# puzzlepaint/surfelmeshing

Measured on AMD Instinct MI355X. Metric: RGB-D frames/s integrated @640x480, 5M live surfels; achieved HBM GB/s, higher is better.
Workload: dtype f32; 1 GPU; C2: synthetic room stream 640x480, raw depth + colour frames resident in HBM, full preprocessing + Integrate per frame, 4912850 live surfels (6250000 slots), steady-state re-traversal; max_surfel_count=6250000, streams=1, parallelism=1 independent stream per GPU

## Files before the change

### surfelmeshing_amd/csrc/smx_recon.hip

```cpp
#include <math.h>
#include <cmath>
#include <stdlib.h>
#include <string.h>

#include <algorithm>
#include <atomic>
#include <vector>

#include "smx_recon_state.hpp"
#include "smx_mesh.hpp"
#include <hip/hip_ext.h>

using namespace smx;

namespace {

struct FrameCtx {
  Mat34 L;
  Mat34 G;
  float fx, fy, cx, cy;
  Unproj up;
  float inv_depth_scaling;
  float sensor_noise_factor;
  float cos_normal_compat;
// ... 634 lines not shown
    have[q] = k < n_binned;
    pr[q] = tb.pairs[(size_t)tile * tb.cap + (have[q] ? k : 0u)];
  }
#pragma unroll
  for (int q = 0; q < kPairCache; ++q) { keep(pr[q].x); keep(pr[q].y); if (!have[q]) pr[q] = make_uint2(0u, 0u); }
  const uint16_t own_depth = in_image ? depth(y, x) : (uint16_t)0;
  const float2 own_normal = in_image ? normals(y, x) : make_float2(0.f, 0.f);
  PairRec rec[kPairCache];
#pragma unroll
  for (int q = 0; q < kPairCache; ++q) rec[q] = fetch_pair(S, c, pr[q].x, pr[q].y);
  t.zmin[lane] = 0x7F800000;
  t.sup[lane] = kInvalid; t.cnt[lane] = 0; t.confl[lane] = kInvalid; t.sum[lane] = 0;
  t.depth[lane] = own_depth; t.nrm[lane] = own_normal;
  __syncthreads();
  SMX_STAMP(stamps, 1);
  auto zmin_stage = [&](const PairRec& r) { if (r.code & kPairActive) atomicMin(&t.zmin[r.code & 255u], __float_as_int(r.l.z)); };
#pragma unroll
  for (int q = 0; q < kPairCache; ++q) if (have[q]) zmin_stage(rec[q]);
  for_uncached_pairs(S, c, tb, tile, n_binned, overflowed, n_ovf, zmin_stage);
  __syncthreads();
  SMX_STAMP(stamps, 2);
  if (lane == 0) {
    tb.count[tile * kCountStride] = 0;
    if (tile == 0) { *next_ovf_count = 0; seg_work_count[0] = 0; seg_work_count[1] = 0; }
    if (c.stats) {
      atomicAdd(&st->n_pairs, n_total);
      atomicMax(&st->max_tile_pairs, n_total);
      if (tile == 0) st->n_overflow_pairs = n_ovf;
    }
  }
#pragma unroll
  for (int q = 0; q < kPairCache; ++q) if (have[q]) assoc_stage(t, c, rec[q]);
  for_uncached_pairs(S, c, tb, tile, n_binned, overflowed, n_ovf, [&](const PairRec& r) { assoc_stage(t, c, r); });
  __syncthreads();
  SMX_STAMP(stamps, 3);
  uint32_t cand[kPairCache];
  float4 cp4[kPairCache], cn4[kPairCache];
#pragma unroll
  for (int q = 0; q < kPairCache; ++q) cand[q] = have[q] ? merge_candidate(t, c, rec[q]) : kInvalid;
#pragma unroll
  for (int q = 0; q < kPairCache; ++q) {
    const uint32_t g = cand[q] == kInvalid ? 0u : cand[q];
    cp4[q] = *S.group(kGroupP, g); cn4[q] = *S.group(kGroupN, g);
  }
#pragma unroll
  for (int q = 0; q < kPairCache; ++q) { keep(cp4[q]); keep(cn4[q]); }
#pragma unroll
  for (int q = 0; q < kPairCache; ++q) if (cand[q] != kInvalid) merge_decide(rec[q], cp4[q], cn4[q], merge_flag);
  for_uncached_pairs(S, c, tb, tile, n_binned, overflowed, n_ovf, [&](const PairRec& r) { merge_stage(t, S, c, r, merge_flag); });
  __syncthreads();
  SMX_STAMP(stamps, 4);
  if (in_image) {
    const size_t k = (size_t)y * c.W + x;
    sc.first_depth[k] = __int_as_float(t.zmin[lane]);
    sc.supporting[k] = t.sup[lane];
    sc.counts[k] = t.cnt[lane];
    sc.depth_sums[k] = (long long)t.sum[lane];
    sc.confl_key[k] = t.confl[lane];
  }
  SMX_STAMP(stamps, 5);
  ts_end(c.ts, kTsTilesEnd, blockIdx.x, gridDim.x);
}

__device__ __forceinline__ float depth_sum_avg(const Scratch& sc, size_t k) {
  return q_to_float(sc.depth_sums[k]) / (float)sc.counts[k];
}

__global__ void __launch_bounds__(kBlock)
k_blend_start(float ds, Img<uint16_t> depth, Scratch sc, BlendBufs b, int W, int H, unsigned long long* ts) {
  ts_end(ts, kTsBlendEnd, blockIdx.y * gridDim.x + blockIdx.x, gridDim.x * gridDim.y);
  const int x = blockIdx.x * 64 + (threadIdx.x & 63);
  const int y = blockIdx.y * 4 + (threadIdx.x >> 6);
  if (!(x >= 1 && y >= 1 && x < W - 1 && y < H - 1)) return;
  const size_t k = (size_t)y * W + x;
  const uint16_t own = depth(y, x);
  if (own == 0 || sc.supporting[k] == kInvalid) return;
  bool measurement_border = false, surfel_border = false;
  for (int wy = y - 1; wy <= y + 1; ++wy)
    for (int wx = x - 1; wx <= x + 1; ++wx) {
      if (depth(wy, wx) == 0) measurement_border = true;
      else if (sc.supporting[(size_t)wy * W + wx] == kInvalid) surfel_border = true;
    }
  if (surfel_border) {
    b.new_distance_map[k] = 1;
    const float avg = depth_sum_avg(sc, k);
    b.new_deltas[k] = avg - (float)own / ds;
  }
  if (measurement_border) {
    b.distance_map[k] = 1;
    const float avg = depth_sum_avg(sc, k);
    b.deltas[k] = avg - (float)own / ds;
    depth(y, x) = f2u16(ds * avg + 0.5f);
  } else {
    b.distance_map[k] = 255;
  }
}

__global__ void __launch_bounds__(kBlock)
k_blend_iter(int it, float term, float ds, Img<uint16_t> depth, Scratch sc, BlendBufs b, int W, int H, unsigned long long* ts) {
  ts_end(ts, kTsBlendEnd, blockIdx.y * gridDim.x + blockIdx.x, gridDim.x * gridDim.y);
  const int x = blockIdx.x * 64 + (threadIdx.x & 63);
  const int y = blockIdx.y * 4 + (threadIdx.x >> 6);
  if (!(x >= 1 && y >= 1 && x < W - 1 && y < H - 1)) return;
  const size_t k = (size_t)y * W + x;
  if (b.distance_map[k] == 255) {
    float delta_sum = 0; int count = 0;
    for (int wy = y - 1; wy <= y + 1; ++wy)
// ... 279 lines not shown
    const int k = min(k0 + j, P - 1);
    const int y = k / W, x = k - y * W;
    dv[j] = depth(y, x); sv[j] = sc.supporting[k]; cv[j] = sc.confl_key[k];
  }
#pragma unroll
  for (int j = 0; j < kScanPxPerThread; ++j) { keep(dv[j]); keep(sv[j]); keep(cv[j]); }
#pragma unroll
  for (int j = 0; j < kScanPxPerThread; ++j) {
    const int k = k0 + j;
    bool fl = false;
    if (k < P) {
      const int y = k / W, x = k - y * W;
      const uint16_t d = (uint16_t)dv[j];
      if (copy_back) depth_out(y, x) = d;
      fl = x >= 1 && y >= 1 && x < W - 1 && y < H - 1 && d > 0 && sv[j] == kInvalid && cv[j] == kInvalid;
      flags[k] = fl ? 1 : 0;
    }
    f[j] = fl ? 1u : 0u;
    mine += f[j];
  }
  const uint32_t lane = threadIdx.x & 63, wave = threadIdx.x >> 6;
  uint32_t incl = mine;
#pragma unroll
  for (int off = 1; off < 64; off <<= 1) {
    const uint32_t t = __shfl_up(incl, off);
    if (lane >= (uint32_t)off) incl += t;
  }
  if (lane == 63) wave_tot[wave] = incl;
  __syncthreads();
  uint32_t wave_off = 0, total = 0;
#pragma unroll
  for (int w = 0; w < kBlock / 64; ++w) {
    if ((uint32_t)w < wave) wave_off += wave_tot[w];
    total += wave_tot[w];
  }
  uint32_t run = wave_off + incl - mine;
#pragma unroll
  for (int j = 0; j < kScanPxPerThread; ++j) {
    const int k = k0 + j;
    if (k < P) local_rank[k] = run;
    run += f[j];
  }
  if (threadIdx.x == 0) {
    block_sums[block] = total;
    if (block == 0) st->create_base_next = st->surfel_count;
  }
}

struct FrameIn {
  Img<const uint16_t> depth; Img<const float2> normals; Img<const float> radius; Img<const uchar3> color;
};

struct PixelIn {
  uint16_t depth; float first; uint32_t key; uint32_t count; float2 nxy; uchar3 col; float radius;
};
__device__ __forceinline__ PixelIn load_pixel(const FrameCtx& c, const Scratch& sc, const FrameIn& in, int x, int y) {
  const size_t k = (size_t)y * c.W + x;
  PixelIn p;
  p.depth = in.depth(y, x); p.first = sc.first_depth[k]; p.key = sc.confl_key[k]; p.count = sc.counts[k];
  p.nxy = in.normals(y, x); p.col = in.color(y, x); p.radius = in.radius(y, x);
  return p;
}

__device__ __forceinline__ void keep(const PixelIn& p) {
  keep((uint32_t)p.depth); keep(p.first); keep(p.key); keep(p.count); keep(p.nxy); keep(p.radius);
  keep((uint32_t)p.col.x | ((uint32_t)p.col.y << 8) | ((uint32_t)p.col.z << 16));
}

struct SurfelRegs {
  float4 P;
  float4 N;
  float4 C;
  bool dirty;
  bool replaced;
  Vec3 new_smooth;
};

__device__ __forceinline__ void integrate_or_conflict(SurfelRegs& R, const FrameCtx& c, const PixelIn& px,
                                                      bool integrate, int x, int y,
                                                      const Vec3& cam, uint32_t i, DevState* st) {
  if (!integrate) return;
  const float measurement_depth = c.inv_depth_scaling * (float)px.depth;
  if (measurement_depth <= 0) return;
  bool conflicting = false;
  const float first = px.first;
  if (first < (1 - c.sensor_noise_factor) * measurement_depth) {
    if (first == cam.z) {
      const uint32_t key = px.key;
      if (key != kInvalid && (key & 0x7FFFFFFFu) == i) conflicting = true;
    }
    integrate = false;
  }
  if (!integrate && !conflicting) return;
  const float occlusion_depth = (1 + c.sensor_noise_factor) * measurement_depth;
  if (cam.z > occlusion_depth) integrate = false;
  if (!integrate && !conflicting) return;

  const float depth = measurement_depth;
  const Vec3 lp = {depth * (c.up.fx_inv * (float)x + c.up.cx_inv), depth * (c.up.fy_inv * (float)y + c.up.cy_inv), depth};
  const Vec3 gp = mul(c.G, lp);
  const float2 nxy = px.nxy;
  const Vec3 mn = {nxy.x, nxy.y, meas_normal_z(nxy.x, nxy.y)};
  const Vec3 gn = rotate(c.G, mn);
  const uchar3 col = px.col;

  if (conflicting) {
    if (c.stats) atomicAdd(&st->n_conflict_hits, 1u);
    float confidence = R.C.x;
    confidence -= 1;
    R.dirty = true;
    if (confidence <= 0) {
      if (c.stats) atomicAdd(&st->n_replaced, 1u);
      R.P = make_float4(gp.x, gp.y, gp.z, __uint_as_float(c.frame));
      R.new_smooth = gp;
      R.replaced = true;
      R.N = make_float4(gn.x, gn.y, gn.z, px.radius);
      R.C = make_float4(1.0f, __uint_as_float(c.frame),
                        __uint_as_float((uint32_t)col.x | ((uint32_t)col.y << 8) | ((uint32_t)col.z << 16) | (1u << 24)), R.C.w);
    } else {
      R.C.x = confidence;
    }
  }
  if (!integrate) return;

  const float surfel_distance = sqrtf(cam.x * cam.x + cam.y * cam.y + cam.z * cam.z);
  const Vec3 sn = {R.N.x, R.N.y, R.N.z};
  const Vec3 ln = rotate(c.L, sn);
  const float dot_angle = (1.0f / surfel_distance) * (cam.x * ln.x + cam.y * ln.y + cam.z * ln.z);
  if (dot_angle > 0) return;
  if (measurement_depth < cam.z) {
    const float d = sn.x * gn.x + sn.y * gn.y + sn.z * gn.z;
    if (d < c.cos_normal_compat) integrate = false;
  }
  const float old_r2 = R.N.w;
  if (old_r2 < 0) integrate = false;
  if (!integrate) return;

  uint32_t cnt = px.count;
  if (cnt < 1) cnt = 1;
  const float weight = 1.0f / (float)cnt;
  if (__float_as_uint(R.C.y) < c.frame) {
    if (c.stats) atomicAdd(&st->n_integrated, 1u);
    const float confidence = R.C.x;
    R.C.x = (confidence + weight < c.max_conf) ? (confidence + weight) : c.max_conf;
    const float nf = 1.0f / (confidence + weight);
    R.P.x = (confidence * R.P.x + weight * gp.x) * nf;
    R.P.y = (confidence * R.P.y + weight * gp.y) * nf;
    R.P.z = (confidence * R.P.z + weight * gp.z) * nf;
    const Vec3 nn = {confidence * sn.x + weight * gn.x, confidence * sn.y + weight * gn.y, confidence * sn.z + weight * gn.z};
    const float inv = 1.0f / sqrtf(nn.x * nn.x + nn.y * nn.y + nn.z * nn.z);
    R.N = make_float4(inv * nn.x, inv * nn.y, inv * nn.z, fminf(old_r2, px.radius));
    const uint32_t oc = __float_as_uint(R.C.z);
    const uint32_t c0 = (uint32_t)(uint8_t)(int)((confidence * (float)(oc & 255u) + weight * (float)col.x) * nf + 0.5f);
    const uint32_t c1 = (uint32_t)(uint8_t)(int)((confidence * (float)((oc >> 8) & 255u) + weight * (float)col.y) * nf + 0.5f);
    const uint32_t c2 = (uint32_t)(uint8_t)(int)((confidence * (float)((oc >> 16) & 255u) + weight * (float)col.z) * nf + 0.5f);
    R.C.z = __uint_as_float(c0 | (c1 << 8) | (c2 << 16));
    R.P.w = __uint_as_float(c.frame);
    R.dirty = true;
  }
}

template <bool kUseList>
__global__ void __launch_bounds__(kBlock)
k_integrate(Surfels S, FrameCtx c, Scratch sc, FrameIn in, Lists L,
            uint8_t* __restrict__ merge_flag, DevState* st, NewFlagsArgs nf, uint32_t n_flag_blocks) {
  SMX_SET_WAVE_PRIO();
#ifdef SMX_STAMPS
  if (nf.dbg && blockIdx.x == 0 && threadIdx.x == 0) nf.dbg[0] = wall_clock64();
#endif
  if (blockIdx.x < n_flag_blocks) { ts_begin(c.ts, kTsIntBegin); new_flags_scan_body(nf, sc, c.W, c.H, st, blockIdx.x); return; }
  const uint32_t block = blockIdx.x - n_flag_blocks, n_blocks = gridDim.x - n_flag_blocks;
  const uint32_t n_scan = kUseList ? 0u : st->surfel_count;
  uint32_t merged_here = 0;
  uint32_t ent, cntv;
  const uint32_t n_steps = vis_begin<kUseList>(L, n_scan, block, ent, cntv);
  for (uint32_t w = block; w < n_steps; w += n_blocks) {
    const uint32_t cur = ent;
    ent = (w + n_blocks < n_steps) ? vis_load<kUseList>(L, w + n_blocks) : 0u;
    uint32_t i;
    if (!vis_entry<kUseList>(cur, w, cntv, n_scan, threadIdx.x, i)) continue;
    const uint32_t merge_mark = merge_flag[i];
    SurfelRegs R;
    R.P = *S.group(kGroupP, i); R.N = *S.group(kGroupN, i); R.C = *S.group(kGroupC, i);
    if (merge_mark) {
      merge_flag[i] = 0;
      S.u(kLastUpdateStamp, i) = 0;
      S.f(kRadiusSq, i) = -1;
      const uint32_t col = (__float_as_uint(R.C.z) & 0x00FFFFFFu) | 0x01000000u;
      S.u(kColor, i) = col;
      L.flags8[i] = make_flags(0u, col, c.frame, c.reg_window);
      L.hot_epoch[i >> L.hot_shift] = (uint8_t)L.epoch;
      if (L.dirty8) L.dirty8[i] = 1;
      ++merged_here;
      continue;
    }
    R.dirty = false; R.replaced = false;
    const float4 p4 = R.P, n4 = R.N;
    if (!is_active(__float_as_uint(p4.w), c.frame, c.window)) continue;
    Proj p;
    const Vec3 g = {p4.x, p4.y, p4.z};
    if (!project_pos(g, c, p)) continue;
    if (n4.w < 0) continue;
    int ox = p.px, oy = p.py;
    const bool second = quadrant(p, c, ox, oy);
    const PixelIn px0 = load_pixel(c, sc, in, p.px, p.py);
    const PixelIn px1 = load_pixel(c, sc, in, ox, oy);
    integrate_or_conflict(R, c, px0, true, p.px, p.py, p.l, i, st);
    integrate_or_conflict(R, c, px1, second, ox, oy, p.l, i, st);
    if (R.dirty) {
      L.hot_epoch[i >> L.hot_shift] = (uint8_t)L.epoch;
      if (L.dirty8) L.dirty8[i] = 1;
      out_store16(S.group(kGroupP, i), R.P); out_store16(S.group(kGroupN, i), R.N);
      out_store16(S.group(kGroupC, i), R.C);
      if (R.replaced) {
        *S.group(kGroupS, i) = make_float4(R.new_smooth.x, R.new_smooth.y, R.new_smooth.z, 0.0f);
        S.set_neighbors(i, make_uint4(kInvalid, kInvalid, kInvalid, kInvalid));
      }
    }
    L.flags8[i] = make_flags(__float_as_uint(R.P.w), __float_as_uint(R.C.z), c.frame, c.reg_window);
  }
#pragma unroll
  for (int off = 32; off > 0; off >>= 1) merged_here += __shfl_xor(merged_here, off);
  if ((threadIdx.x & 63) == 0 && merged_here) {
    atomicAdd(&st->merge_count, merged_here);
    if (c.stats) atomicAdd(&st->n_merged, merged_here);
  }
  ts_end(c.ts, kTsIntEnd, block, min(n_blocks, n_steps));
}

template <bool kUseList>
__device__ __forceinline__ void update_neighbors_body(const Surfels& S, const FrameCtx& c, const Scratch& sc, const FrameIn& in,
                                                      const Lists& L, const DevState* st, uint32_t block, uint32_t n_blocks) {
  const int kDX[4] = {-1, 1, 0, 0}, kDY[4] = {0, 0, -1, 1};
  const uint32_t n_scan = kUseList ? 0u : st->create_base_next;
  if (block == 0 && threadIdx.x < kSubLists) { L.rec_chunks.count[threadIdx.x * kCountStride] = 0; L.acc_chunks.count[threadIdx.x * kCountStride] = 0; }
  uint32_t ent, cntv;
  const uint32_t n_steps = vis_begin<kUseList>(L, n_scan, block, ent, cntv);
  for (uint32_t w = block; w < n_steps; w += n_blocks) {
    const uint32_t cur = ent;
    ent = (w + n_blocks < n_steps) ? vis_load<kUseList>(L, w + n_blocks) : 0u;
    uint32_t i;
    if (!vis_entry<kUseList>(cur, w, cntv, n_scan, threadIdx.x, i)) continue;
    const float4 p4 = *S.group(kGroupP, i), n4 = *S.group(kGroupN, i);
    const uint4 t4 = *reinterpret_cast<const uint4*>(S.group(kGroupT, i));
    if (!is_active(__float_as_uint(p4.w), c.frame, c.window)) continue;
    const Vec3 g = {p4.x, p4.y, p4.z};
    const Vec3 cam = mul(c.L, g);
    if (!(cam.z > 0)) continue;
    const float u = c.fx * (cam.x / cam.z) + c.cx, v = c.fy * (cam.y / cam.z) + c.cy;
    if (!(u >= 1.0f && v >= 1.0f && u < (float)(c.W - 1) && v < (float)(c.H - 1))) continue;
    const int x = (int)u, y = (int)v;
    const float measurement_depth = c.inv_depth_scaling * (float)in.depth(y, x);
    const float obs_r2 = in.radius(y, x);
    uint32_t cand[4];
#pragma unroll
    for (int d = 0; d < 4; ++d) cand[d] = sc.supporting[(size_t)(y + kDY[d]) * c.W + (x + kDX[d])];
    const float occlusion_depth = (1 + c.sensor_noise_factor) * measurement_depth;
    if (cam.z > occlusion_depth) continue;
    const float surfel_distance = sqrtf(cam.x * cam.x + cam.y * cam.y + cam.z * cam.z);
// ... 833 lines not shown
  }
  uint32_t total;
  (void)block_excl_scan(mine, wave_tot, total);
  if (threadIdx.x == 0) seg_count[blockIdx.x] = total;
}
__global__ void __launch_bounds__(1024)
k_delta_scan(uint32_t* __restrict__ seg_count, int nseg, uint32_t* __restrict__ total_out) {
  __shared__ uint32_t wave_tot[1024 / 64];
  __shared__ uint32_t carry;
  if (threadIdx.x == 0) carry = 0;
  __syncthreads();
  for (int base = 0; base < nseg; base += 1024) {
    const int b = base + threadIdx.x;
    const uint32_t v = (b < nseg) ? seg_count[b] : 0;
    uint32_t total;
    const uint32_t excl = block_excl_scan<1024 / 64>(v, wave_tot, total);
    if (b < nseg) seg_count[b] = carry + excl;
    __syncthreads();
    if (threadIdx.x == 0) carry += total;
    __syncthreads();
  }
  if (threadIdx.x == 0) *total_out = carry;
}
__global__ void __launch_bounds__(kBlock)
k_delta_gather(Surfels S, uint8_t* __restrict__ dirty8, const uint32_t* __restrict__ seg_offset, float* __restrict__ out,
               uint32_t total, const DevState* st) {
  __shared__ uint32_t wave_tot[kBlock / 64];
  const uint32_t N = st->surfel_count, i0 = blockIdx.x * kSeg + threadIdx.x * 4;
  uint32_t bits = 0;
  if (i0 < N) {
    const uchar4 d = *reinterpret_cast<const uchar4*>(&dirty8[i0]);
    bits = (d.x != 0 ? 1u : 0u) | ((i0 + 1 < N && d.y != 0) ? 2u : 0u) | ((i0 + 2 < N && d.z != 0) ? 4u : 0u) |
           ((i0 + 3 < N && d.w != 0) ? 8u : 0u);
    if (bits) *reinterpret_cast<uchar4*>(&dirty8[i0]) = make_uchar4(0, 0, 0, 0);
  }
  uint32_t seg_total;
  uint32_t off = seg_offset[blockIdx.x] + block_excl_scan((uint32_t)__popc(bits), wave_tot, seg_total);
  const int want[8] = {kSmoothX, kSmoothY, kSmoothZ, kRadiusSq, kNormalX, kNormalY, kNormalZ, kLastUpdateStamp};
#pragma unroll
  for (int j = 0; j < 4; ++j)
    if (bits & (1u << j)) {
      const uint32_t i = i0 + j;
      out[off] = __uint_as_float(i);
#pragma unroll
      for (int k = 0; k < 8; ++k) out[(size_t)(k + 1) * total + off] = S.f(want[k], i);
      ++off;
    }
}

__global__ void __launch_bounds__(kBlock)
k_decode_conflicting(const uint32_t* __restrict__ key, uint32_t* __restrict__ out, int P) {
  const int k = blockIdx.x * kBlock + threadIdx.x;
  if (k < P) out[k] = (key[k] == kInvalid) ? kInvalid : (key[k] & 0x7FFFFFFFu);
}

__global__ void __launch_bounds__(kBlock)
k_global_ranks(const uint32_t* __restrict__ local_rank, const uint32_t* __restrict__ block_offsets,
               uint32_t* __restrict__ out, int P) {
  const int k = blockIdx.x * kBlock + threadIdx.x;
  if (k < P) out[k] = block_offsets[k / kScanPxPerBlock] + local_rank[k];
}

}

enum : int {
  kSlotScanVisible = 0, kSlotAssocTiles, kSlotBlend, kSlotIntegrate,
  kSlotUpdateNeighbors, kSlotNeighborScan,
  kSlotRegAccumulate, kSlotRegStep,
  kSlotRegUpdate,
  kSlotCull,
  kSlotEmpty,
  kSlotCount
};
static const char* const kSlotNames[kSlotCount] = {
  "scan_visible", "assoc_tiles", "blend", "integrate+new_flags", "update_neighbors+create",
  "neighbor_scan", "reg_accumulate", "reg_step", "reg_update", "cull_segments", "empty_slot"};

struct SlotTimer {
  smx_recon r; hipStream_t st; int slot; bool kev, prof, by_launch;
  SlotTimer(smx_recon r_, hipStream_t st_, int slot_, bool launch_carries = false) : r(r_), st(st_), slot(slot_) {
    kev = (r->timing_enabled & 2) != 0;
    prof = (r->prof_slot == slot) && r->prof_ev && r->prof_n < r->prof_cap;
    by_launch = prof && launch_carries;
    if (kev) (void)hipEventRecord(r->kev[2 * slot], st);
    if (prof && !by_launch) (void)hipEventRecord(r->prof_ev[2 * r->prof_n], st);
  }
  hipEvent_t start() const { return by_launch ? r->prof_ev[2 * r->prof_n] : nullptr; }
  hipEvent_t stop() const { return by_launch ? r->prof_ev[2 * r->prof_n + 1] : nullptr; }
  ~SlotTimer() {
    if (kev) { (void)hipEventRecord(r->kev[2 * slot + 1], st); r->kev_recorded[slot] = true; }
    if (prof) { if (!by_launch) (void)hipEventRecord(r->prof_ev[2 * r->prof_n + 1], st); r->prof_n++; }
  }
};

namespace {

int enqueue_regularize(smx_recon r, hipStream_t st, uint32_t frame, float rf, float weight, int window,
                       bool detach, bool copy_only, bool zero_chunks, unsigned long long* ts = nullptr, hipEvent_t acc_done = nullptr) {
  const dim3 g(r->nsegB), bB(kBlockB), gl(r->grid_list), b(kBlock);
  const float rf2 = rf * rf;
  if (!r->table_valid || r->table_frame != frame || r->table_window != window) {
    hipLaunchKernelGGL(k_rebuild_flags, dim3(r->grid_surfels), b, 0, st, r->S, frame, window, r->L.flags8, r->st);
    r->table_valid = true; r->table_frame = frame; r->table_window = window;
    r->hot_holdoff = 3;
    SMX_HIP(hipMemsetAsync(r->L.seg_streak, 0, (size_t)r->nseg, st));
  }
// ... 122 lines not shown
  r->nsegB = div_up((long long)r->S.pitch, kSegB);
  r->fb.cap = kFarBinCap; r->fb.hash_mask = (uint32_t)kFarHash - 1u;
  SMX_TRY(r->mem.alloc(&r->fb.rec, (size_t)r->nsegB * kFarBinCap, false));
  SMX_TRY(r->mem.alloc(&r->fb.count, ((size_t)r->nsegB + 1) * kCountStride, true));
  r->L.vis_region = (uint32_t)(div_up(r->nseg, kSubLists) * kSeg);
  SMX_TRY(r->mem.alloc(&r->L.vis_list, (size_t)kSubLists * r->L.vis_region, true));
  SMX_TRY(r->mem.alloc(&r->L.recent_list, (size_t)r->nsegB * kSegB, false));
  SMX_TRY(r->mem.alloc(&r->L.vis_seg, (size_t)r->nseg, true));
  SMX_TRY(r->mem.alloc(&r->L.seg_box, (size_t)r->nseg * 8, true));
  SMX_TRY(r->mem.alloc(&r->L.seg_act, (size_t)r->nseg, true));
  SMX_TRY(r->mem.alloc(&r->L.seg_streak, (size_t)r->nseg, true));
  SMX_TRY(r->mem.alloc(&r->sw.surv_list, (size_t)r->nseg + 65536, true));
  SMX_TRY(r->mem.alloc(&r->sw.copy_list, (size_t)r->nseg + 65536, true));
  SMX_TRY(r->mem.alloc(&r->sw.count, 2, true));
  SMX_TRY(r->mem.alloc_host(&r->dir_host, 2, true));
  r->dir_host[0] = 0;
  r->dir_host[1] = 0;
  SMX_TRY(hip_rc(hipHostGetDevicePointer(reinterpret_cast<void**>(&r->dir_dev), r->dir_host, 0), "hipHostGetDevicePointer"));
  SMX_TRY(r->mem.alloc(&r->L.recent_seg, (size_t)r->nsegB, true));
  r->L.vis_chunks.stride = 0; r->L.vis_chunks.desc = nullptr;
  r->L.rec_chunks.stride = (uint32_t)(div_up(r->nsegB, kSubLists) + 8192);
  SMX_TRY(r->mem.alloc(&r->L.rec_chunks.desc, (size_t)kSubLists * r->L.rec_chunks.stride, true));
  SMX_TRY(r->mem.alloc(&r->L.rec_chunks.count, (size_t)kSubLists * kCountStride, true));
  static_assert(kSegAcc == kSegB && kAccCount < kCountStride, "pass B lists the edge kernel's segments by its own segment numbers");
  r->L.acc_chunks.stride = r->L.rec_chunks.stride;
  r->L.acc_chunks.count = r->L.rec_chunks.count + kAccCount;
  SMX_TRY(r->mem.alloc(&r->L.acc_chunks.desc, (size_t)kSubLists * r->L.acc_chunks.stride, true));
  SMX_TRY(r->mem.alloc(&r->flags_buf[0], (size_t)r->nsegB * kSegB, true));
  SMX_TRY(r->mem.alloc(&r->flags_buf[1], (size_t)r->nsegB * kSegB, true));
  r->L.flags8 = r->flags_buf[0];
  r->L.hot_shift = 10;
  while ((((size_t)r->nseg * kSeg) >> r->L.hot_shift) + 1 > (size_t)kMaxHotGroups) ++r->L.hot_shift;
  r->L.n_hot_groups = (uint32_t)((((size_t)r->nseg * kSeg) >> r->L.hot_shift) + 1);
  SMX_TRY(r->mem.alloc(&r->L.hot_epoch, (size_t)r->L.n_hot_groups + 64, true));
  SMX_TRY(r->mem.alloc(&r->L.seg_targets, (size_t)r->nsegB * kBlockB, true));
  r->L.epoch = 128;
  r->hot_filter_enabled = 1;
  r->fuse_edges = kFuseEdgesDefault;
  r->hot_holdoff = 3;
  SMX_TRY(r->mem.alloc(&r->merge_flag, r->S.pitch, true));
  SMX_TRY(r->mem.alloc(&r->gate_count, 32, true));
  r->gate_expected = 0;
  constexpr int kHandoverModeDefault = 1;
  r->handover_mode = kHandoverModeDefault;
  {
    const char* cc = getenv("ROCPROF_COUNTER_COLLECTION");
    if (cc && cc[0] && strcmp(cc, "0") != 0) r->handover_mode = 0;
  }
  SMX_TRY(r->mem.alloc(&r->L.act_list, (size_t)r->nsegB * kSegB, true));
  SMX_TRY(r->mem.alloc(&r->sc.supporting, P, true));
  SMX_TRY(r->mem.alloc(&r->sc.counts, P, true));
  SMX_TRY(r->mem.alloc(&r->sc.depth_sums, P, true));
  SMX_TRY(r->mem.alloc(&r->sc.confl_key, P, true));
  SMX_TRY(r->mem.alloc(&r->sc.first_depth, P, true));
  for (int k = 0; k < 2; ++k) {
    SMX_TRY(r->mem.alloc(&r->vis_count_set[k], (size_t)kSubLists * kCountStride, true));
    SMX_TRY(r->mem.alloc(&r->ovf_count_set[k], 1, true));
  }
  r->L.vis_chunks.count = r->vis_count_set[0];
  r->tb.tiles_x = div_up(width, kTileW);
  r->tb.n_tiles = (uint32_t)(r->tb.tiles_x * div_up(height, kTileH));
  r->tb.cap = r->bin_cap_full = kTileBinCap;
  SMX_TRY(r->mem.alloc(&r->tb.pairs, (size_t)r->tb.n_tiles * kTileBinCap, false));
  SMX_TRY(r->mem.alloc(&r->tb.count, (size_t)r->tb.n_tiles * kCountStride, true));
  SMX_TRY(r->mem.alloc(&r->tb.ovf, 2 * (size_t)r->S.pitch + 64, false));
  r->tb.ovf_count = r->ovf_count_set[0];
#ifdef SMX_STAMPS
  SMX_TRY(r->mem.alloc(&r->stamps, (size_t)3 * 16 * 8192, true));
#endif
  SMX_TRY(r->mem.alloc(&r->blended_depth, P, true));
  SMX_TRY(r->mem.alloc(&r->bb.distance_map, P, true));
  SMX_TRY(r->mem.alloc(&r->bb.new_distance_map, P, true));
  SMX_TRY(r->mem.alloc(&r->bb.deltas, P, true));
  SMX_TRY(r->mem.alloc(&r->bb.new_deltas, P, true));
  SMX_TRY(r->mem.alloc(&r->new_flags, P, true));
  SMX_TRY(r->mem.alloc(&r->new_ranks, P, true));
  SMX_TRY(r->mem.alloc(&r->tmp_u32, P, true));
  r->n_scan_blocks = div_up((long long)P, kScanPxPerBlock);
  SMX_TRY(r->mem.alloc(&r->block_sums, (size_t)r->n_scan_blocks, true));
  SMX_TRY(r->mem.alloc(&r->block_offsets, (size_t)r->n_scan_blocks, true));
  SMX_TRY(r->mem.alloc(&r->st, 1, true));
  SMX_TRY(r->mem.alloc(&r->ts_ring, (size_t)kTsRing * kTsWords, true));
  SMX_TRY(r->mem.alloc_host(&r->ts_host, (size_t)kTsRing * kTsWords, false));
  SMX_TRY(r->mem.alloc_host(&r->ts_mapped, (size_t)kTsRing * kTsWords, true));
  memset(const_cast<unsigned long long*>(r->ts_mapped), 0, sizeof(unsigned long long) * kTsRing * kTsWords);
  SMX_TRY(hip_rc(hipHostGetDevicePointer(reinterpret_cast<void**>(&r->ts_mapped_dev), const_cast<unsigned long long*>(r->ts_mapped), 0), "hipHostGetDevicePointer"));
  SMX_TRY(hip_rc(hipDeviceGetAttribute(&r->wall_khz, hipDeviceAttributeWallClockRate, device), "hipDeviceGetAttribute"));
  if (r->wall_khz <= 0) r->wall_khz = 100000;
  for (int i = 0; i < 14; ++i) SMX_TRY(hip_rc(hipEventCreate(&r->ev[i]), "hipEventCreate"));
  for (int i = 0; i < 2 * 16; ++i) SMX_TRY(hip_rc(hipEventCreate(&r->kev[i]), "hipEventCreate"));
  {
    int lo = 0, hi = 0;
    SMX_TRY(hip_rc(hipDeviceGetStreamPriorityRange(&lo, &hi), "hipDeviceGetStreamPriorityRange"));
    SMX_TRY(hip_rc(hipStreamCreateWithPriority(&r->reg_stream, hipStreamNonBlocking, hi), "hipStreamCreateWithPriority"));
  }
  const unsigned evf = hipEventDisableTiming | hipEventReleaseToDevice;
  SMX_TRY(hip_rc(hipEventCreateWithFlags(&r->ev_front, evf), "hipEventCreateWithFlags"));
  SMX_TRY(hip_rc(hipEventCreateWithFlags(&r->ev_upd, evf), "hipEventCreateWithFlags"));
  SMX_TRY(hip_rc(hipEventCreateWithFlags(&r->ev_reg, evf), "hipEventCreateWithFlags"));
  r->overlap_enabled = 1;
  r->prof_slot = -1;
  r->timing_enabled = 4;
  hipDeviceProp_t prop;
  SMX_TRY(hip_rc(hipGetDeviceProperties(&prop, device), "hipGetDeviceProperties"));
#undef SMX_TRY
  const int cus = prop.multiProcessorCount > 0 ? prop.multiProcessorCount : 256;
  r->grid_surfels = cus * 8;
// ... 134 lines not shown
  SMX_CHECK_ARG(radius->width == r->W && radius->height == r->H && color->width == r->W && color->height == r->H);
  SMX_CHECK_ARG(!p->do_blending || (p->measurement_blending_radius >= 2 && p->measurement_blending_radius <= 255));
  hipStream_t st = (hipStream_t)s;
  if (r->have_frame && (int32_t)(frame_index - r->last_frame) < 0) {
    SMX_CALL(join_regularizer(r, st));
    SMX_HIP(hipMemsetAsync(r->L.vis_seg, 0, (size_t)r->nseg * 4, st));
    SMX_HIP(hipMemsetAsync(r->L.seg_box, 0, (size_t)r->nseg * 8 * sizeof(float), st));
    r->hot_holdoff = 3;
  }
  r->have_frame = true; r->last_frame = frame_index;
  if (r->handover_mode == 1 && reinterpret_cast<volatile uint32_t*>(r->dir_host)[1] != 0u) r->handover_mode = 0;
  FrameCtx c;
  memcpy(c.G.m, global_T_local, sizeof(float) * 12);
  c.L = se3_inverse(global_T_local);
  c.fx = r->fx; c.fy = r->fy; c.cx = r->cx; c.cy = r->cy;
  c.up = make_unproj(r->fx, r->fy, r->cx, r->cy);
  c.inv_depth_scaling = 1.0f / depth_scaling;
  c.sensor_noise_factor = p->sensor_noise_factor;
  c.cos_normal_compat = cosf((float)(M_PI / 180.0f * p->normal_compatibility_threshold_deg));
  c.rf2 = p->radius_factor_for_regularization_neighbors * p->radius_factor_for_regularization_neighbors;
  c.max_conf = p->max_surfel_confidence;
  c.window = p->surfel_integration_active_window_size;
  c.reg_window = p->regularization_frame_window_size;
  c.frame = frame_index;
  c.W = r->W; c.H = r->H;
  c.stats = r->stats_enabled;
  c.ts = nullptr;
  if (r->timing_enabled & 4) { ++r->ts_seq; c.ts = r->ts_ring + (size_t)(r->ts_seq % kTsRing) * kTsWords; }
  const int P = r->W * r->H;
  const dim3 b(kBlock), gpx(div_up(P, kBlock)), gimg(div_up(r->W, 64), div_up(r->H, 4));
  const dim3 gs(r->nseg), gl(r->grid_list);
  const bool tm = (r->timing_enabled & 1) != 0;
  FrameIn in;
  in.depth = as_img<const uint16_t>(depth); in.normals = as_img<const float2>(normals);
  in.radius = as_img<const float>(radius); in.color = as_img<const uchar3>(color);
  const Img<uint16_t> depth_rw = as_img<uint16_t>(depth);

  const uint8_t* flags_prev = r->L.flags8;
  r->L.flags8 = (r->L.flags8 == r->flags_buf[0]) ? r->flags_buf[1] : r->flags_buf[0];
  r->L.epoch = (r->L.epoch + 1u) & 255u;
  if (r->hot_holdoff > 0) --r->hot_holdoff;
  const bool pipelined = r->overlap_enabled != 0;
  const hipStream_t sF = st;
  const hipStream_t sR = pipelined ? r->reg_stream : st;
  const bool split = pipelined && (r->debug_skip & 16) != 0;
  if (r->reg_pending && r->last_stream != st) SMX_CALL(join_regularizer(r, st));
  r->last_stream = st;
  if (r->stats_enabled) hipLaunchKernelGGL(k_reset_frame_stats, dim3(1), dim3(1), 0, sF, r->st, 1);
  if (tm) SMX_HIP(hipEventRecord(r->ev[0], sF));
  r->L.descending = *reinterpret_cast<volatile uint32_t*>(r->dir_host);
  r->sc_cur ^= 1;
  r->L.vis_chunks.count = r->vis_count_set[r->sc_cur];
  r->tb.ovf_count = r->ovf_count_set[r->sc_cur];
  if (hook_ready) SMX_HIP(hipStreamWaitEvent(sF, hook_ready, 0));
  {
    SlotTimer t(r, sF, kSlotCull);
    if (r->sw_dirty) SMX_HIP(hipMemsetAsync(r->sw.count, 0, 2 * sizeof(uint32_t), sF));
    r->sw_dirty = true;
    hipLaunchKernelGGL(k_cull_segments, dim3((unsigned)div_up(r->nseg, kBlock)), b, 0, sF, c, r->L, r->sw, r->st, (uint32_t)r->nseg, (uint32_t)P, r->ts_seq); }
  if (r->pending_mark) { SMX_HIP(hipStreamWaitEvent(sF, r->pending_mark, 0)); r->pending_mark = nullptr; }
  if (r->stats_enabled) hipLaunchKernelGGL(k_reset_frame_stats, dim3(1), dim3(1), 0, sF, r->st, 0);
  { SlotTimer t(r, sF, kSlotScanVisible, true);
    const bool lds_tables = !r->no_lds_tables;
    constexpr int kPassAWgsPerCu = 8;
    const dim3 ga((unsigned)(r->cu_count * kPassAWgsPerCu));
    hipExtLaunchKernelGGL(k_scan_visible, ga, b, 0, sF, t.start(), t.stop(), 0, r->S, c, r->L, r->tb, r->sw, flags_prev, r->st, lds_tables ? 1 : 0);
    r->table_valid = true; r->table_frame = frame_index; r->table_window = c.reg_window; }
  { SlotTimer t(r, sF, kSlotAssocTiles, true);
    hipExtLaunchKernelGGL(k_assoc_tiles, dim3(r->tb.n_tiles), dim3(kTilePx), 0, sF, t.start(), t.stop(), 0, r->S, c, r->sc, in.depth, in.normals, r->tb,
                       r->ovf_count_set[r->sc_cur ^ 1], r->merge_flag, r->st, r->L.seg_act, (uint32_t)r->nseg, r->dir_dev, r->sw.count,
                       r->stamps ? r->stamps : nullptr, r->ts_ring, c.ts ? r->ts_mapped_dev : nullptr, r->ts_seq);
    r->sw_dirty = false; }
  if (tm) { SMX_HIP(hipEventRecord(r->ev[1], sF)); SMX_HIP(hipEventRecord(r->ev[2], sF)); SMX_HIP(hipEventRecord(r->ev[3], sF)); SMX_HIP(hipEventRecord(r->ev[4], sF)); }
  const int halo = p->measurement_blending_radius - 1;
  const bool fused_blend = p->do_blending && halo <= kBlendMaxHalo && !r->blend_multi_launch;
  bool front_by_launch = false, front_by_gate = false;
  const float ds = 1.0f / c.inv_depth_scaling;
  const float term = p->do_blending ? 1.0f / ((float)p->measurement_blending_radius - 1.0f) : 0.0f;
  const Img<uint16_t> blended = {r->blended_depth, r->H, r->W, (size_t)r->W * sizeof(uint16_t)};
  if (fused_blend) {
    front_by_gate = pipelined && !split && r->handover_mode == 1 && !(r->debug_skip & 4) && !tm && !(r->timing_enabled & 2);
    SlotTimer t(r, sF, kSlotBlend, front_by_gate);
    const int cus = r->cu_count;
    int tile = 32;
    if (40 + 2 * halo <= 64) {
      auto cost = [&](int t) { const long long n = (long long)div_up(r->W, t) * div_up(r->H, t); return ((n + cus - 1) / cus) * (long long)(t + 2 * halo) * (t + 2 * halo); };
      if ((cost(40) < cost(32)) != (r->blend_other_tile != 0)) tile = 40;
    }
    const int rw = tile + 2 * halo;
    const size_t lds = sizeof(BlendMasks) + (size_t)rw * rw * 10;
    const int tiles_x = div_up(r->W, tile);
    const uint32_t n_blend = (uint32_t)(tiles_x * div_up(r->H, tile));
    unsigned long long* stamps = (r->stamps && (frame_index & 63u) == 32u) ? r->stamps + 16 * 8192 : nullptr;
    front_by_launch = !front_by_gate && pipelined && !split && !tm && !(r->timing_enabled & 2) && r->prof_slot != kSlotBlend;
    uint32_t* const gate = front_by_gate ? r->gate_count : nullptr;
    if (front_by_gate) r->gate_expected += n_blend;
    const hipEvent_t start = front_by_gate ? t.start() : nullptr;
    const hipEvent_t stop = front_by_gate ? t.stop() : front_by_launch ? r->ev_front : nullptr;
    if (tile == 40)
      hipExtLaunchKernelGGL(k_blend_tiles<40>, dim3(n_blend), dim3(kBlendThreads), (uint32_t)lds, sF, start, stop, 0, p->measurement_blending_radius, term, ds,
                            in.depth, blended, r->sc, r->W, r->H, tiles_x, stamps, c.ts, gate, (r->debug_skip & 256) ? 1 : kBlendMaxRings);
    else
      hipExtLaunchKernelGGL(k_blend_tiles<32>, dim3(n_blend), dim3(kBlendThreads), (uint32_t)lds, sF, start, stop, 0, p->measurement_blending_radius, term, ds,
                            in.depth, blended, r->sc, r->W, r->H, tiles_x, stamps, c.ts, gate, (r->debug_skip & 256) ? 1 : kBlendMaxRings);
  } else if (p->do_blending) {
    SlotTimer t(r, sF, kSlotBlend);
    SMX_HIP(hipMemsetAsync(r->bb.distance_map, 0, (size_t)P, sF));
    SMX_HIP(hipMemsetAsync(r->bb.new_distance_map, 0, (size_t)P, sF));
    hipLaunchKernelGGL(k_blend_start, gimg, b, 0, sF, ds, depth_rw, r->sc, r->bb, r->W, r->H, c.ts);
    for (int it = 2; it < p->measurement_blending_radius; ++it)
      hipLaunchKernelGGL(k_blend_iter, gimg, b, 0, sF, it, term, ds, depth_rw, r->sc, r->bb, r->W, r->H, c.ts);
  }
// ... 260 lines not shown
  } else if (!enabled && r->L.dirty8) {
    r->L.dirty8 = nullptr;
    r->dirty.reset();
  }
  return SMX_OK;
}

int smx_recon_transfer_changed_to_cpu(smx_recon r, smx_stream s, uint32_t frame_index, smx_surfel_delta_cpu* d) {
  SMX_CHECK_ARG(r != nullptr && d != nullptr);
  SMX_ON_DEVICE(r->device);
  if (!r->L.dirty8) { set_error("delta tracking is off (smx_recon_set_delta_tracking)"); return SMX_ERR_INVALID_ARGUMENT; }
  hipStream_t st = (hipStream_t)s;
  SMX_CALL(join_regularizer(r, st));
  hipLaunchKernelGGL(k_delta_count, dim3(r->nseg), dim3(kBlock), 0, st, r->L.dirty8, r->delta_seg.get(), r->st);
  enqueue_segment_scan(st, r->delta_seg.get(), r->nseg, r->delta_total.get());
  SMX_LAUNCH_CHECK();
  uint32_t total = 0, n = 0;
  SMX_HIP(hipMemcpyAsync(&total, r->delta_total.get(), 4, hipMemcpyDeviceToHost, st));
  SMX_HIP(hipMemcpyAsync(&n, &r->st->surfel_count, 4, hipMemcpyDeviceToHost, st));
  SMX_HIP(hipStreamSynchronize(st));
  d->frame_index = frame_index;
  d->surfel_count = n;
  d->count = total;
  if (total > d->capacity) {
    set_error("delta of %u slots does not fit the capacity %u", total, d->capacity);
    return SMX_ERR_INVALID_ARGUMENT;
  }
  if (total == 0) return SMX_OK;
  SMX_CHECK_ARG(d->surfel_index && d->x && d->y && d->z && d->radius_squared && d->normal_x && d->normal_y &&
                d->normal_z && d->last_update_stamp);
  SMX_CALL(acquire_staging(r, st, (size_t)9 * total));
  hipLaunchKernelGGL(k_delta_gather, dim3(r->nseg), dim3(kBlock), 0, st, r->S, r->L.dirty8, r->delta_seg.get(), r->staging.buf.get(), total,
                     r->st);
  SMX_LAUNCH_CHECK();
  void* dst[9] = {d->surfel_index, d->x, d->y, d->z, d->radius_squared, d->normal_x, d->normal_y, d->normal_z,
                  d->last_update_stamp};
  for (int k = 0; k < 9; ++k)
    SMX_HIP(hipMemcpyAsync(dst[k], r->staging.buf.get() + (size_t)k * total, (size_t)total * 4, hipMemcpyDeviceToHost, st));
  SMX_HIP(hipStreamSynchronize(st));
  return SMX_OK;
}

int smx_recon_debug_download_scratch(smx_recon r, smx_stream s, int32_t which, void* dst) {
  SMX_CHECK_ARG(r != nullptr && dst != nullptr);
  SMX_ON_DEVICE(r->device);
  SMX_CALL(join_regularizer(r, (hipStream_t)s));
  hipStream_t st = (hipStream_t)s;
  const size_t P = (size_t)r->W * r->H;
  const void* src = nullptr; size_t bytes = 0;
  switch (which) {
    case SMX_SCRATCH_SUPPORTING: src = r->sc.supporting; bytes = P * 4; break;
    case SMX_SCRATCH_SUPPORT_COUNTS: src = r->sc.counts; bytes = P * 4; break;
    case SMX_SCRATCH_DEPTH_SUMS: src = r->sc.depth_sums; bytes = P * 8; break;
    case SMX_SCRATCH_FIRST_DEPTH: src = r->sc.first_depth; bytes = P * 4; break;
    case SMX_SCRATCH_NEW_FLAGS: src = r->new_flags; bytes = P; break;
    case SMX_SCRATCH_CONFLICTING:
      hipLaunchKernelGGL(k_decode_conflicting, dim3(div_up((long long)P, kBlock)), dim3(kBlock), 0, st, r->sc.confl_key, r->tmp_u32, (int)P);
      src = r->tmp_u32; bytes = P * 4; break;
    case SMX_SCRATCH_NEW_INDICES:
      hipLaunchKernelGGL(k_global_ranks, dim3(div_up((long long)P, kBlock)), dim3(kBlock), 0, st, r->new_ranks, r->block_offsets, r->tmp_u32, (int)P);
      src = r->tmp_u32; bytes = P * 4; break;
    default: set_error("unknown scratch id %d", which); return SMX_ERR_INVALID_ARGUMENT;
  }
  SMX_HIP(hipMemcpyAsync(dst, src, bytes, hipMemcpyDeviceToHost, st));
  SMX_HIP(hipStreamSynchronize(st));
  return SMX_OK;
}

int smx_recon_debug_count_skipped_segments(smx_recon r, smx_stream s, uint32_t* out) {
  SMX_CHECK_ARG(r != nullptr && out != nullptr);
  SMX_ON_DEVICE(r->device);
  SMX_CALL(join_regularizer(r, (hipStream_t)s));
  std::vector<uint32_t> marks((size_t)r->nsegB);
  SMX_HIP(hipMemcpyAsync(marks.data(), r->L.recent_seg, marks.size() * 4, hipMemcpyDeviceToHost, (hipStream_t)s));
  SMX_HIP(hipStreamSynchronize((hipStream_t)s));
  uint32_t n = 0;
  for (uint32_t m : marks) n += m == kInvalid ? 1u : 0u;
  *out = n;
  return SMX_OK;
}

}
```

### surfelmeshing_amd/csrc/smx_recon_state.hpp

```cpp
#pragma once

#include "smx_common.hpp"
#include "smx_components.hpp"
#include "smx_decimate.hpp"
#include "smx_distance.hpp"
#include "smx_fill.hpp"
#include "smx_raycast.hpp"
#include "smx_render.hpp"
#include "smx_track.hpp"

namespace smx {

struct MeshWorkspace;

enum : int {
  kX = 0, kY = 1, kZ = 2, kSmoothX = 3, kSmoothY = 4, kSmoothZ = 5, kConfidence = 6, kRadiusSq = 7,
  kNormalX = 8, kNormalY = 9, kNormalZ = 10, kGradX = 11, kGradY = 12, kGradZ = 13,
  kCreationStamp = 17, kLastUpdateStamp = 18, kNeighbor0 = 19, kGradCount = 23, kColor = 24, kRows = 25
};

struct DevState {
  uint32_t surfel_count;
  uint32_t merge_count;
  uint32_t create_base_next;
  uint32_t recent_count;
  uint32_t create_base;
  uint32_t new_count;
  uint32_t capacity_clamped;
  uint32_t n_visible, n_merged, n_edges, n_integrated, n_replaced, n_conflict_hits;
  uint32_t n_window_edges, n_contributors;
  uint32_t n_segments_skipped;
  uint32_t reg_saturated;
  uint32_t n_pairs, n_overflow_pairs, max_tile_pairs;
};

enum : int { kGroupP = 0, kGroupS, kGroupN, kGroupT, kGroupC, kGroupG, kGroups };
__host__ __device__ constexpr int row_group(int row) {
  return row <= 2 ? kGroupP : row <= 5 ? kGroupS : row == 6 ? kGroupC : row == 7 ? kGroupN : row <= 10 ? kGroupN
       : row <= 13 ? kGroupG : row <= 16 ? -1 : row == 17 ? kGroupC : row == 18 ? kGroupP : row <= 22 ? kGroupT
       : row == 24 ? kGroupC : -1;
}
__host__ __device__ constexpr int row_sub(int row) {
  return row <= 2 ? row : row <= 5 ? row - 3 : row == 6 ? 0 : row == 7 ? 3 : row <= 10 ? row - 8
       : row <= 13 ? row - 11 : row == 17 ? 1 : row == 18 ? 3 : row <= 22 ? row - 19 : row == 24 ? 2 : -1;
}
__host__ __device__ constexpr int group_start(int g) { return g; }
constexpr int kQuadsPerSlot = 6;
struct Surfels {
  float* base;
  size_t pitch;
  __host__ __device__ __forceinline__ size_t quad(int g, uint32_t i) const { return (size_t)group_start(g) * pitch + (size_t)i; }
  __device__ __forceinline__ float& f(int row, uint32_t i) const { return base[quad(row_group(row), i) * 4 + row_sub(row)]; }
  __device__ __forceinline__ uint32_t& u(int row, uint32_t i) const {
    return reinterpret_cast<uint32_t*>(base)[quad(row_group(row), i) * 4 + row_sub(row)];
  }
  __device__ __forceinline__ float4* group(int g, uint32_t i) const { return reinterpret_cast<float4*>(base) + quad(g, i); }
  __device__ __forceinline__ void set_neighbors(uint32_t i, const uint4& t) const { *reinterpret_cast<uint4*>(group(kGroupT, i)) = t; }
  __device__ __forceinline__ void set_neighbor(uint32_t i, int q, uint32_t v) const { u(kNeighbor0 + q, i) = v; }
  struct View { const float4* p; size_t stride; };
  View view(int g) const { return View{reinterpret_cast<const float4*>(base) + quad(g, 0), quad(g, 1) - quad(g, 0)}; }
};

struct Scratch {
  uint32_t* supporting;
  uint32_t* counts;
  long long* depth_sums;
  uint32_t* confl_key;
  float* first_depth;
};

constexpr int kBlock = 256;

constexpr int kSeg = 1024;
constexpr int kSegB = 1024;
constexpr int kBlockB = kSegB / 4;
constexpr uint32_t kCountStride = 32;
constexpr uint32_t kSubLists = 16;
struct Chunks { uint32_t* desc; uint32_t* count; uint32_t stride; };
struct Lists {
  Chunks vis_chunks, rec_chunks;
  Chunks acc_chunks;
  uint32_t* vis_list;
  uint32_t vis_region;
  float* seg_box;
  uint32_t* vis_seg;
  uint8_t* seg_streak;
  uint32_t* recent_list;
  uint32_t* recent_seg;
  uint32_t* act_list;
  uint8_t* flags8;
  uint8_t* dirty8;
  uint8_t* seg_act;
  uint32_t descending;
  uint8_t* hot_epoch;
  uint16_t* seg_targets;
  uint32_t n_hot_groups;
  uint32_t epoch;
  int hot_shift;
};

struct FarBins {
  uint4* rec;
  uint32_t* count;
  uint32_t cap;
  uint32_t hash_mask;
};

struct TileBins {
  uint2* pairs;
  uint32_t* count;
  uint4* ovf;
  uint32_t* ovf_count;
  uint32_t cap;
  int tiles_x;
  uint32_t n_tiles;
};

template <int kWaves = kBlock / 64>
__device__ __forceinline__ uint32_t block_excl_scan(uint32_t mine, uint32_t* wave_tot , uint32_t& total) {
  const uint32_t lane = threadIdx.x & 63, wave = threadIdx.x >> 6;
  uint32_t incl = mine;
// ... 48 lines not shown
    const uint32_t red = vis_u8(255.99f * blend);
    return vis_rgb(red, 255u - red, 80u);
  }
  if (vc.flags & SMX_VIS_NORMALS) {
    const float4 n = *S.group(kGroupN, i);
    return vis_rgb(vis_u8(255.99f / 2.0f * (n.x + 1.0f)), vis_u8(255.99f / 2.0f * (n.y + 1.0f)),
                   vis_u8(255.99f / 2.0f * (n.z + 1.0f)));
  }
  return S.u(kColor, i);
}

struct StagingWork { DevBuf<float> buf; StreamMark mark; };
struct CompactWork { DevBuf<uint32_t> map, seg, out; };
struct CandidateWork { DevBuf<float> q; DevBuf<uint32_t> slots; DevBuf<uint8_t> state; };

}

struct smx_recon_s {
  smx::DevBlocks mem;
  int device;
  uint32_t max_surfels;
  int W, H;
  float fx, fy, cx, cy;
  smx::Surfels S;
  long long* grad_acc;
  float4* reg_rec;
  smx::FarBins fb;
  smx::Lists L;
  int nseg;
  int nsegB;
  uint8_t* merge_flag;
  bool table_valid;
  uint32_t table_frame;
  int table_window;
  int stats_enabled;
  hipEvent_t hook_consumed, hook_chain;
  hipEvent_t hook_ready;
  int blend_multi_launch;
  smx::Scratch sc;
  smx::TileBins tb;
  smx::SegWork sw;
  bool sw_dirty;
  hipEvent_t pending_mark;
  uint32_t* ovf_count_set[2];
  unsigned long long* stamps;
  int no_lds_tables;
  int blend_other_tile;
  int cu_count;
  uint32_t bin_cap_full;
  uint32_t* vis_count_set[2];
  uint32_t* dir_host;
  uint32_t* dir_dev;
  int sc_cur;
  int hot_holdoff;
  int hot_filter_enabled;
  int fuse_edges;
  uint16_t* blended_depth;
  smx::BlendBufs bb;
  uint8_t* new_flags;
  uint32_t* new_ranks;
  uint32_t* block_sums;
  uint32_t* block_offsets;
  uint32_t* tmp_u32;
  int n_scan_blocks;
  smx::DevState* st;
  int scan_mode;
  int timing_enabled;
  bool have_timings;
  unsigned long long* ts_ring;
  unsigned long long* ts_host;
  volatile unsigned long long* ts_mapped;
  unsigned long long* ts_mapped_dev;
  unsigned long long ts_seq;
  int wall_khz;
  hipEvent_t ev[14];
  hipEvent_t kev[2 * 16];
  bool kev_recorded[16];
  int prof_slot;
  int prof_cap, prof_n;
  hipEvent_t* prof_ev;
  smx::DevBuf<uint8_t> dirty;
  smx::DevBuf<uint32_t> delta_seg;
  smx::DevBuf<uint32_t> delta_total;
  int grid_surfels;
  int grid_list;
  int grid_acc;
  int grid_list_full;
  int debug_skip;
  int overlap_enabled;
  hipStream_t reg_stream;
  uint32_t* gate_count;
  uint32_t gate_expected;
  int handover_mode;
  hipEvent_t ev_front;
  hipEvent_t ev_upd;
  hipEvent_t ev_reg;
  bool reg_pending;
  hipStream_t last_stream;
  uint8_t* flags_buf[2];
  bool have_frame;
  uint32_t last_frame;
  smx::StagingWork staging;
  smx::RenderWork render;
  smx::TrackWork track;
  smx::DecimateWork decimate;
  smx::ComponentsWork components;
// ... 19 lines not shown
```

Baseline: 6103 frames/s.

## Pack per-pixel association and static inputs into 16-byte records for surfel gather

```diff
diff --git a/surfelmeshing_amd/csrc/smx_recon.hip b/surfelmeshing_amd/csrc/smx_recon.hip
--- a/surfelmeshing_amd/csrc/smx_recon.hip
+++ b/surfelmeshing_amd/csrc/smx_recon.hip
@@ -710,7 +710,7 @@
   SMX_STAMP(stamps, 4);
   if (in_image) {
     const size_t k = (size_t)y * c.W + x;
-    sc.first_depth[k] = __int_as_float(t.zmin[lane]);
+    sc.px_assoc[k] = make_uint4((uint32_t)t.zmin[lane], t.confl[lane], t.cnt[lane], t.sup[lane]);
     sc.supporting[k] = t.sup[lane];
     sc.counts[k] = t.cnt[lane];
     sc.depth_sums[k] = (long long)t.sum[lane];
@@ -1096,19 +1096,32 @@
 };
 
 struct PixelIn {
-  uint16_t depth; float first; uint32_t key; uint32_t count; float2 nxy; uchar3 col; float radius;
+  uint16_t depth; float first; uint32_t key; uint32_t count; float2 nxy; uint32_t col ; float radius;
 };
-__device__ __forceinline__ PixelIn load_pixel(const FrameCtx& c, const Scratch& sc, const FrameIn& in, int x, int y) {
+__device__ __forceinline__ PixelIn load_pixel(const FrameCtx& c, const uint4* __restrict__ px_assoc, const float4* __restrict__ px_static,
+                                              const FrameIn& in, int x, int y) {
   const size_t k = (size_t)y * c.W + x;
   PixelIn p;
-  p.depth = in.depth(y, x); p.first = sc.first_depth[k]; p.key = sc.confl_key[k]; p.count = sc.counts[k];
-  p.nxy = in.normals(y, x); p.col = in.color(y, x); p.radius = in.radius(y, x);
+  p.depth = in.depth(y, x);
+  const uint4 a = px_assoc[k];
+  const float4 s = px_static[k];
+  p.first = __uint_as_float(a.x); p.key = a.y; p.count = a.z;
+  p.nxy = make_float2(s.x, s.y); p.radius = s.z; p.col = __float_as_uint(s.w);
   return p;
 }
-
 __device__ __forceinline__ void keep(const PixelIn& p) {
-  keep((uint32_t)p.depth); keep(p.first); keep(p.key); keep(p.count); keep(p.nxy); keep(p.radius);
-  keep((uint32_t)p.col.x | ((uint32_t)p.col.y << 8) | ((uint32_t)p.col.z << 16));
+  keep((uint32_t)p.depth); keep(p.first); keep(p.key); keep(p.count); keep(p.nxy); keep(p.radius); keep(p.col);
+}
+
+__global__ void __launch_bounds__(kBlock)
+k_pack_pixels(Img<const float2> normals, Img<const float> radius, Img<const uchar3> color, float4* __restrict__ out, int W, int H) {
+  const int x = blockIdx.x * 64 + (threadIdx.x & 63);
+  const int y = blockIdx.y * 4 + (threadIdx.x >> 6);
+  if (x >= W || y >= H) return;
+  const float2 n = normals(y, x);
+  const uchar3 col = color(y, x);
+  out[(size_t)y * W + x] = make_float4(n.x, n.y, radius(y, x),
+                                       __uint_as_float((uint32_t)col.x | ((uint32_t)col.y << 8) | ((uint32_t)col.z << 16)));
 }
 
 struct SurfelRegs {
@@ -1146,7 +1159,7 @@
   const float2 nxy = px.nxy;
   const Vec3 mn = {nxy.x, nxy.y, meas_normal_z(nxy.x, nxy.y)};
   const Vec3 gn = rotate(c.G, mn);
-  const uchar3 col = px.col;
+  const uchar3 col = make_uchar3((unsigned char)(px.col & 255u), (unsigned char)((px.col >> 8) & 255u), (unsigned char)((px.col >> 16) & 255u));
 
   if (conflicting) {
     if (c.stats) atomicAdd(&st->n_conflict_hits, 1u);
@@ -1247,8 +1260,9 @@
     if (n4.w < 0) continue;
     int ox = p.px, oy = p.py;
     const bool second = quadrant(p, c, ox, oy);
-    const PixelIn px0 = load_pixel(c, sc, in, p.px, p.py);
-    const PixelIn px1 = load_pixel(c, sc, in, ox, oy);
+    const PixelIn px0 = load_pixel(c, sc.px_assoc, sc.px_static, in, p.px, p.py);
+    const PixelIn px1 = load_pixel(c, sc.px_assoc, sc.px_static, in, ox, oy);
+    keep(px0); keep(px1);
     integrate_or_conflict(R, c, px0, true, p.px, p.py, p.l, i, st);
     integrate_or_conflict(R, c, px1, second, ox, oy, p.l, i, st);
     if (R.dirty) {
@@ -2188,6 +2202,12 @@
 k_decode_conflicting(const uint32_t* __restrict__ key, uint32_t* __restrict__ out, int P) {
   const int k = blockIdx.x * kBlock + threadIdx.x;
   if (k < P) out[k] = (key[k] == kInvalid) ? kInvalid : (key[k] & 0x7FFFFFFFu);
+}
+
+__global__ void __launch_bounds__(kBlock)
+k_decode_first_depth(const uint4* __restrict__ px_assoc, uint32_t* __restrict__ out, int P) {
+  const int k = blockIdx.x * kBlock + threadIdx.x;
+  if (k < P) out[k] = px_assoc[k].x;
 }
 
 __global__ void __launch_bounds__(kBlock)
@@ -2416,7 +2436,9 @@
   SMX_TRY(r->mem.alloc(&r->sc.counts, P, true));
   SMX_TRY(r->mem.alloc(&r->sc.depth_sums, P, true));
   SMX_TRY(r->mem.alloc(&r->sc.confl_key, P, true));
-  SMX_TRY(r->mem.alloc(&r->sc.first_depth, P, true));
+  SMX_TRY(r->mem.alloc(&r->sc.px_assoc, P, true));
+  for (int k = 0; k < 2; ++k) SMX_TRY(r->mem.alloc(&r->px_static_set[k], P, true));
+  r->sc.px_static = r->px_static_set[0];
   for (int k = 0; k < 2; ++k) {
     SMX_TRY(r->mem.alloc(&r->vis_count_set[k], (size_t)kSubLists * kCountStride, true));
     SMX_TRY(r->mem.alloc(&r->ovf_count_set[k], 1, true));
@@ -2657,12 +2679,14 @@
   r->sc_cur ^= 1;
   r->L.vis_chunks.count = r->vis_count_set[r->sc_cur];
   r->tb.ovf_count = r->ovf_count_set[r->sc_cur];
+  r->sc.px_static = r->px_static_set[r->sc_cur];
   if (hook_ready) SMX_HIP(hipStreamWaitEvent(sF, hook_ready, 0));
   {
     SlotTimer t(r, sF, kSlotCull);
     if (r->sw_dirty) SMX_HIP(hipMemsetAsync(r->sw.count, 0, 2 * sizeof(uint32_t), sF));
     r->sw_dirty = true;
     hipLaunchKernelGGL(k_cull_segments, dim3((unsigned)div_up(r->nseg, kBlock)), b, 0, sF, c, r->L, r->sw, r->st, (uint32_t)r->nseg, (uint32_t)P, r->ts_seq); }
+  hipLaunchKernelGGL(k_pack_pixels, gimg, b, 0, sF, in.normals, in.radius, in.color, r->px_static_set[r->sc_cur], r->W, r->H);
   if (r->pending_mark) { SMX_HIP(hipStreamWaitEvent(sF, r->pending_mark, 0)); r->pending_mark = nullptr; }
   if (r->stats_enabled) hipLaunchKernelGGL(k_reset_frame_stats, dim3(1), dim3(1), 0, sF, r->st, 0);
   { SlotTimer t(r, sF, kSlotScanVisible, true);
@@ -3029,7 +3053,9 @@
     case SMX_SCRATCH_SUPPORTING: src = r->sc.supporting; bytes = P * 4; break;
     case SMX_SCRATCH_SUPPORT_COUNTS: src = r->sc.counts; bytes = P * 4; break;
     case SMX_SCRATCH_DEPTH_SUMS: src = r->sc.depth_sums; bytes = P * 8; break;
-    case SMX_SCRATCH_FIRST_DEPTH: src = r->sc.first_depth; bytes = P * 4; break;
+    case SMX_SCRATCH_FIRST_DEPTH:
+      hipLaunchKernelGGL(k_decode_first_depth, dim3(div_up((long long)P, kBlock)), dim3(kBlock), 0, st, r->sc.px_assoc, r->tmp_u32, (int)P);
+      src = r->tmp_u32; bytes = P * 4; break;
     case SMX_SCRATCH_NEW_FLAGS: src = r->new_flags; bytes = P; break;
     case SMX_SCRATCH_CONFLICTING:
       hipLaunchKernelGGL(k_decode_conflicting, dim3(div_up((long long)P, kBlock)), dim3(kBlock), 0, st, r->sc.confl_key, r->tmp_u32, (int)P);
diff --git a/surfelmeshing_amd/csrc/smx_recon_state.hpp b/surfelmeshing_amd/csrc/smx_recon_state.hpp
--- a/surfelmeshing_amd/csrc/smx_recon_state.hpp
+++ b/surfelmeshing_amd/csrc/smx_recon_state.hpp
@@ -66,7 +66,8 @@
   uint32_t* counts;
   long long* depth_sums;
   uint32_t* confl_key;
-  float* first_depth;
+  uint4* px_assoc;
+  const float4* px_static;
 };
 
 constexpr int kBlock = 256;
@@ -221,6 +222,7 @@
   uint32_t* dir_host;
   uint32_t* dir_dev;
   int sc_cur;
+  float4* px_static_set[2];
   int hot_holdoff;
   int hot_filter_enabled;
   int fuse_edges;
```

Result: no change. 6146 frames/s (median of 6 runs) (+0.7%).
